# deepreinforce-ai/CUDA-L2

Measured on NVIDIA H100. Metric: HGEMM TFLOP/s, offline mode, per (M,N,K), higher is better.
Workload: dtype f16 x f16 -> f32 accumulate -> f16

## Files before the change

cuda_l2_b200/csrc/hgemm_sm90.cuh:

```cuda
#pragma once
#include <cuda.h>
#include <cuda_runtime.h>
#include <cstdint>

#include "hgemm_schedule.cuh"
#include "ptx_sm90.cuh"
#include "wgmma_sm90.cuh"


namespace b200 {

constexpr int kBlockKBytes = 128;
constexpr int kBlockK = 64;
constexpr int kWgmmaK = 16;
constexpr int kBlockM = 128;
constexpr int kNumThreads = 384;
constexpr int kEpiWarp0 = 4;
constexpr int kConsumerThreads = 256;
constexpr int kProducerRegs = 40;
constexpr int kConsumerRegs = 232;
constexpr int kSmemLimit = 232448;
enum KMode : int { kPlain = 0, kWorkspaceSplitK = 1, kClusterSplitK = 2, kStreamK = 3 };

template <int BN_, int STAGES_, int CTA_GROUP_, bool ACC_F32_, int CLUSTER_M_ = 1, int CLUSTER_N_ = 1, int M_REP_ = 1, bool BF16_ = false,
          bool E4M3_ = false>
struct Config {
  static constexpr int BN = BN_;
  static constexpr int CTA_GROUP = CTA_GROUP_;
  static constexpr bool ACC_F32 = ACC_F32_;
  static constexpr bool BF16 = BF16_;
  static_assert(!BF16_ || ACC_F32_, "bf16 operands accumulate in fp32");
  static constexpr bool E4M3 = E4M3_;
  static_assert(!E4M3_ || ACC_F32_, "e4m3 operands accumulate in fp32");
  static constexpr int OP_BYTES = E4M3_ ? 1 : 2;
  static constexpr int BLOCK_K = kBlockKBytes / OP_BYTES;
  static constexpr int CLUSTER_M = CLUSTER_M_;
  static constexpr int CLUSTER_N = CLUSTER_N_;
  static constexpr int MCAST_CTAS = CLUSTER_M * CLUSTER_N;
  static constexpr int MCAST_M = CTA_GROUP * CLUSTER_M;
  static constexpr int CLUSTER_CTAS = MCAST_M * CLUSTER_N;
  static constexpr int M_REP = M_REP_;
  static constexpr int CTA_M = kBlockM * M_REP;
  static constexpr int TILE_M = CTA_M * CTA_GROUP;
  static constexpr int A_BOX_ROWS = CTA_M / CLUSTER_N;
  static constexpr int B_BOX_ROWS = BN / MCAST_M;
  static constexpr int A_STAGE_BYTES = CTA_M * kBlockK * 2;
  static constexpr int B_STAGE_BYTES = BN * kBlockK * 2;
  static constexpr int STAGE_BYTES = A_STAGE_BYTES + B_STAGE_BYTES;
  static constexpr int EPI_N = BN < 64 ? BN : 64;
  static constexpr int EPI_CHUNKS = BN / EPI_N;
  static constexpr int EPI_ROWS = 16;
  static constexpr int NUM_THREADS = kNumThreads;
  static constexpr bool STREAM_K = CLUSTER_M_ * CLUSTER_N_ == 1 && BN_ >= 64 && M_REP_ == 1;
  static constexpr bool SPLIT_K = STREAM_K && CTA_GROUP_ == 1;
  static constexpr bool BLOCK_SCALED = false, BATCHED = false, GROUPED = false, ROW_MAJOR_B = false;
  using Cursor = NoBatches;
  static constexpr int EPI_BYTES = 8 * EPI_ROWS * 64 * 2;
  static constexpr int BAR_BYTES = 256;
  static constexpr int MAX_STAGES = (kSmemLimit - 1024 - EPI_BYTES - BAR_BYTES) / STAGE_BYTES;
  static constexpr int STAGES = STAGES_ < MAX_STAGES ? STAGES_ : MAX_STAGES;
  static constexpr int SMEM_BYTES = 1024  + STAGES * STAGE_BYTES + EPI_BYTES + BAR_BYTES;
  static_assert(BN == 32 || BN % 64 == 0, "tile N is 32 or a multiple of 64");
  static_assert(BN >= 32 && BN <= 256, "wgmma N constraints");
  static_assert(M_REP * BN <= 256, "register accumulators: at most 256 columns x 128 rows per consumer warpgroup");
  static_assert(CLUSTER_CTAS <= 8, "portable cluster size");
  static_assert(A_BOX_ROWS % 8 == 0 && B_BOX_ROWS % 8 == 0, "slices must cover whole 8-row swizzle atoms");
  static_assert(M_REP == 1 || M_REP == 2, "one or two 128-row blocks per CTA");
  static_assert(A_BOX_ROWS <= 256 && B_BOX_ROWS <= 256, "TMA box dimension limit");
  static_assert(STAGES >= 2, "the ring needs two stages");
  static_assert(SMEM_BYTES <= kSmemLimit, "exceeds 227 KB of shared memory");
  static_assert(A_STAGE_BYTES % 1024 == 0 && B_STAGE_BYTES % 1024 == 0, "swizzle-128B tiles need 1 KB alignment");
  static_assert(8 * (2 * STAGES + 1) <= BAR_BYTES, "barrier block too small");
};

constexpr int kMaxSplitTiles = 256;

template <class Base>
struct BlockScaled : Base {
  static constexpr bool BLOCK_SCALED = true;
  static_assert(Base::E4M3 && Base::M_REP * Base::BN <= 128, "block scales: e4m3, and room for two accumulator sets");
  static constexpr int SA_WINDOW_BYTES = Base::CTA_M * 4;
  static constexpr int SCALE_STAGE_BYTES = SA_WINDOW_BYTES + 16;
  static constexpr int MAX_STAGES =
      (kSmemLimit - 1024 - Base::EPI_BYTES - Base::BAR_BYTES) / (Base::STAGE_BYTES + SCALE_STAGE_BYTES);
  static constexpr int STAGES = Base::STAGES < MAX_STAGES ? Base::STAGES : MAX_STAGES;
  static constexpr int SMEM_BYTES = Base::SMEM_BYTES + STAGES * SCALE_STAGE_BYTES - (Base::STAGES - STAGES) * Base::STAGE_BYTES;
  static_assert(STAGES >= 2 && SMEM_BYTES <= kSmemLimit, "block-scaled ring does not fit");
};
template <class Cfg>
__host__ __device__ constexpr bool block_scaled() { return Cfg::BLOCK_SCALED; }

template <class Base>
struct Batched : Base {
  static constexpr bool BATCHED = true;
  using Cursor = BatchCursor;
  static_assert(!Base::E4M3, "batched: 16-bit operands, or block-scaled e4m3 (Batched<BlockScaled<...>>)");
};
template <class Base>
struct Batched<BlockScaled<Base>> : BlockScaled<Base> {
  static constexpr bool BATCHED = true;
  using Cursor = BatchCursor;
};
template <class Cfg>
__host__ __device__ constexpr bool batched() { return Cfg::BATCHED; }

template <class Base>
struct Grouped : Base {
  static constexpr bool GROUPED = true;
  using Cursor = GroupCursor;
  static_assert(!Base::E4M3, "grouped: 16-bit operands, or block-scaled e4m3 (Grouped<BlockScaled<...>>)");
};
template <class Base>
struct Grouped<BlockScaled<Base>> : BlockScaled<Base> {
  static constexpr bool GROUPED = true;
  using Cursor = GroupCursor;
  static constexpr int SA_WINDOW_BYTES = Base::CTA_M * 4 + 16;
  static constexpr int SCALE_STAGE_BYTES = SA_WINDOW_BYTES + 16;
  static constexpr int MAX_STAGES =
      (kSmemLimit - 1024 - Base::EPI_BYTES - Base::BAR_BYTES) / (Base::STAGE_BYTES + SCALE_STAGE_BYTES);
  static constexpr int STAGES = Base::STAGES < MAX_STAGES ? Base::STAGES : MAX_STAGES;
  static constexpr int SMEM_BYTES = Base::SMEM_BYTES + STAGES * SCALE_STAGE_BYTES - (Base::STAGES - STAGES) * Base::STAGE_BYTES;
  static_assert(STAGES >= 2 && SMEM_BYTES <= kSmemLimit, "grouped block-scaled ring does not fit");
  static_assert(Base::CTA_M % 4 == 0, "the scale window's shift is the group's");
};
template <class Cfg>
__host__ __device__ constexpr bool grouped() { return Cfg::GROUPED; }

template <class Base>
struct RowMajorB : Base {
  static constexpr bool ROW_MAJOR_B = true;
  static_assert(!Base::E4M3 && !Base::BLOCK_SCALED && !Base::BATCHED && !Base::GROUPED,
                "row-major B: the 2-D 16-bit kernels only");
  static_assert(Base::BN % 64 == 0, "row-major B: whole 64-column atom columns");
  static constexpr int B_ATOMS = Base::BN / 64;
  static constexpr int B_ATOM_BYTES = 64 * kBlockK * 2;
  static constexpr int B_K_ROWS = kBlockK / Base::MCAST_M;
  static_assert(B_K_ROWS % 8 == 0, "K slices of whole 8-row swizzle groups");
  static_assert(B_ATOMS * B_ATOM_BYTES == Base::B_STAGE_BYTES, "the stage holds the same bytes as the K-major one");
};
template <class Cfg>
__host__ __device__ constexpr bool row_major_b() { return Cfg::ROW_MAJOR_B; }

struct Scales { const float* a; const float* b; bool rowwise = false; };

template <class Cfg>
__device__ __forceinline__ float output_scale(const Scales& s) {
  if constexpr (Cfg::E4M3 && !block_scaled<Cfg>()) return s.rowwise ? 1.f : __fmul_rn(*s.a, *s.b);
  else return 1.f;
}

template <class Cfg>
__device__ __forceinline__ void scale_quad(float4& acc, float scale, const Scales& s, int gm, int gn) {
  if constexpr (Cfg::E4M3 && !block_scaled<Cfg>()) {
    if (s.rowwise) {
      const float sa = s.a[gm];
      const float4 sb = *reinterpret_cast<const float4*>(s.b + gn);
      acc.x = __fmul_rn(__fmul_rn(acc.x, sb.x), sa); acc.y = __fmul_rn(__fmul_rn(acc.y, sb.y), sa);
      acc.z = __fmul_rn(__fmul_rn(acc.z, sb.z), sa); acc.w = __fmul_rn(__fmul_rn(acc.w, sb.w), sa);
    } else {
      acc.x = __fmul_rn(acc.x, scale); acc.y = __fmul_rn(acc.y, scale);
      acc.z = __fmul_rn(acc.z, scale); acc.w = __fmul_rn(acc.w, scale);
    }
  }
}

struct RowwiseEpi { float sa_lo, sa_hi; const float* sb; };

__device__ __forceinline__ int frag_row(int lane, int p) { return (lane >> 2) + 8 * (p & 1); }
__device__ __forceinline__ int frag_col(int lane, int p) { return (p >> 1) * 8 + (lane & 3) * 2; }

template <class Cfg, class Reg, int NR>
__device__ __forceinline__ float2 acc_pair(const Reg (&d)[NR], int p) {
  if constexpr (Cfg::ACC_F32) {
    return make_float2(d[2 * p], d[2 * p + 1]);
  } else {
    const uint32_t v = d[p];
    const __half2 h = *reinterpret_cast<const __half2*>(&v);
    return make_float2(__low2float(h), __high2float(h));
  }
}
template <class Cfg, class Reg, int NR>
__device__ __forceinline__ uint32_t acc_packed(const Reg (&d)[NR], int p) {
  if constexpr (Cfg::ACC_F32) return ptx::pack_out_x2_rn<Cfg::BF16>(d[2 * p], d[2 * p + 1]);
  else return d[p];
}

template <class Cfg, class Reg, int NR>
__device__ __forceinline__ void epilogue_store_chunk(const Reg (&d)[NR], int chunk, uint32_t epi_buf, int lane,
                                                     const CUtensorMap* tmap_c, int col0, int row0, int M, int N,
                                                     const RowwiseEpi* rw = nullptr, int batch = 0,
                                                     __half* __restrict__ c_raw = nullptr) {
  using namespace ptx;
  constexpr int EN = Cfg::EPI_N;
  constexpr int PER_CHUNK = EN / 4;
  if (lane == 0) tma_store_wait_read<0>();
  __syncwarp();
  [[maybe_unused]] float2 sb_lane = make_float2(0.f, 0.f);
  [[maybe_unused]] float sbx = 0.f, sby = 0.f;
  if constexpr (Cfg::E4M3) {
    const int n = col0 + 2 * lane;
    if (rw && 2 * lane < EN && n < N) sb_lane = *reinterpret_cast<const float2*>(rw->sb + n);
  }
#pragma unroll
  for (int q = 0; q < PER_CHUNK; ++q) {
    uint32_t off = uint32_t(frag_row(lane, q) * (EN * 2) + frag_col(lane, q) * 2);
    off ^= (EN == 64 ? ((off >> 7) & 7u) : ((off >> 7) & 3u)) << 4;
    if constexpr (Cfg::E4M3) {
      if (rw) {
        if ((q & 1) == 0) {
          const int src = frag_col(lane, q) / 2;
          sbx = __shfl_sync(0xffffffffu, sb_lane.x, src);
          sby = __shfl_sync(0xffffffffu, sb_lane.y, src);
        }
        const float sa = (q & 1) ? rw->sa_hi : rw->sa_lo;
        const float2 v = acc_pair<Cfg>(d, chunk * PER_CHUNK + q);
        st_shared_b32(epi_buf + off, pack_out_x2_rn<Cfg::BF16>(__fmul_rn(__fmul_rn(v.x, sbx), sa),
                                                               __fmul_rn(__fmul_rn(v.y, sby), sa)));
        continue;
      }
    }
    st_shared_b32(epi_buf + off, acc_packed<Cfg>(d, chunk * PER_CHUNK + q));
  }
  fence_proxy_async_smem();
  __syncwarp();
  if constexpr (grouped<Cfg>()) {
    if (row0 + Cfg::EPI_ROWS > M) {
      constexpr int CPR = EN * 2 / 16;
#pragma unroll 1
      for (int i = lane; i < Cfg::EPI_ROWS * CPR; i += 32) {
        const int r = i / CPR, c = i % CPR;
        if (row0 + r < M && col0 + 8 * c < N) {
          uint32_t off = uint32_t(r * (EN * 2) + c * 16);
          off ^= (EN == 64 ? ((off >> 7) & 7u) : ((off >> 7) & 3u)) << 4;
          *reinterpret_cast<uint4*>(c_raw + size_t(row0 + r) * N + col0 + 8 * c) = ld_shared_v4_b32(epi_buf + off);
        }
      }
      return;
    }
  }
  if (lane == 0) {
    if (row0 < M && col0 < N) {
      if constexpr (batched<Cfg>()) tma_store_3d(tmap_c, epi_buf, col0, row0, batch);
      else tma_store_2d(tmap_c, epi_buf, col0, row0);
    }
    tma_store_commit();
  }
}

template <class Cfg, class Reg, int NR>
__device__ __forceinline__ void splitk_epilogue(const Reg (&d)[NR], int e, int row_base, int lane, int tile, int split,
                                                int splits, int m_base, int n0, int M, int N, float* __restrict__ ws,
                                                unsigned* __restrict__ ctr, __half* __restrict__ C,
                                                uint32_t red_smem, uint32_t red_bar, const Scales& scales) {
  using namespace ptx;
  constexpr int BN = Cfg::BN;
  float* slot = ws + (size_t(tile) * splits + split) * (kBlockM * BN);
#pragma unroll
  for (int p = 0; p < NR * (Cfg::ACC_F32 ? 1 : 2) / 2; ++p) {
    const float2 v = acc_pair<Cfg>(d, p);
    __stcg(reinterpret_cast<float2*>(slot + size_t(row_base + frag_row(lane, p)) * BN + frag_col(lane, p)), v);
  }
  __threadfence();
  asm volatile("bar.sync 1, %0;" ::"n"(kConsumerThreads) : "memory");
  if (e == 0) {
    asm volatile("red.release.gpu.global.add.u32 [%0], 1;" ::"l"(ctr + tile) : "memory");
    unsigned seen = 0, spins = 0;
    do {
      asm volatile("ld.acquire.gpu.global.u32 %0, [%1];" : "=r"(seen) : "l"(ctr + tile) : "memory");
      if (seen < unsigned(splits)) {
        __nanosleep(64);
        if (++spins > (1u << 24)) __trap();
      }
    } while (seen < unsigned(splits));
  }
  asm volatile("bar.sync 1, %0;" ::"n"(kConsumerThreads) : "memory");
  const int rows_per = (kBlockM + splits - 1) / splits;
  const int r0 = split * rows_per;
  const int r1 = min(kBlockM, r0 + rows_per);
  if (r0 < r1) {
    const uint32_t slice_bytes = uint32_t(r1 - r0) * BN * 4u;
    const float* tile_ws = ws + size_t(tile) * splits * (kBlockM * BN) + size_t(r0) * BN;
    if (e == 0) {
      fence_proxy_async_all();
      mbar_arrive_expect_tx(red_bar, slice_bytes * uint32_t(splits));
      for (int sp = 0; sp < splits; ++sp)
        bulk_load_1d(red_smem + uint32_t(sp) * slice_bytes, tile_ws + size_t(sp) * (kBlockM * BN), slice_bytes, red_bar);
    }
    mbar_wait(red_bar, 0);
    const float scale = output_scale<Cfg>(scales);
    constexpr int V = BN / 4;
    for (int i = e; i < (r1 - r0) * V; i += kConsumerThreads) {
      const int r = r0 + i / V, c4 = i % V;
      const int gm = m_base + r, gn = n0 + c4 * 4;
      if (gm >= M || gn >= N) continue;
      float4 acc = make_float4(0.f, 0.f, 0.f, 0.f);
      for (int sp = 0; sp < splits; ++sp) {
        const float4 p = ld_shared_v4f(red_smem + uint32_t(sp) * slice_bytes + uint32_t(i) * 16u);
        acc.x += p.x; acc.y += p.y; acc.z += p.z; acc.w += p.w;
      }
      scale_quad<Cfg>(acc, scale, scales, gm, gn);
      uint2 out;
      out.x = pack_out_x2_rn<Cfg::BF16>(acc.x, acc.y);
      out.y = pack_out_x2_rn<Cfg::BF16>(acc.z, acc.w);
      *reinterpret_cast<uint2*>(C + size_t(gm) * N + gn) = out;
    }
  }
  asm volatile("bar.sync 1, %0;" ::"n"(kConsumerThreads) : "memory");
  if (e == 0) {
    unsigned old;
    asm volatile("atom.acq_rel.gpu.global.add.u32 %0, [%1], 1;" : "=r"(old) : "l"(ctr + kMaxSplitTiles + tile) : "memory");
    if (old == unsigned(splits - 1)) {
      ctr[tile] = 0;
      ctr[kMaxSplitTiles + tile] = 0;
      __threadfence();
    }
  }
}

__host__ __device__ constexpr uint32_t cluster_partial_row_bytes(int bn) { return uint32_t(bn) * 4u + 16u; }

template <class Cfg, class Reg, int NR>
__device__ __forceinline__ void cluster_splitk_park(const Reg (&d)[NR], int row_base, int lane, uint32_t part_smem) {
  using namespace ptx;
#pragma unroll
  for (int p = 0; p < NR * (Cfg::ACC_F32 ? 1 : 2) / 2; ++p) {
    const float2 v = acc_pair<Cfg>(d, p);
    st_shared_v2f(part_smem + uint32_t(row_base + frag_row(lane, p)) * cluster_partial_row_bytes(Cfg::BN) +
                      uint32_t(frag_col(lane, p)) * 4u, v.x, v.y);
  }
}

template <class Cfg>
__device__ __forceinline__ void cluster_splitk_reduce(int e, int split, int splits, int m_base, int n0, int M, int N,
                                                      uint32_t part_smem, __half* __restrict__ C,
                                                      const Scales& scales) {
  using namespace ptx;
  constexpr int BN = Cfg::BN;
  constexpr int V = BN / 4;
  const float scale = output_scale<Cfg>(scales);
  const int rows_per = kBlockM / splits;
  const int r0 = split * rows_per;
  uint32_t peer[8];
#pragma unroll
  for (int p = 0; p < 8; ++p) peer[p] = (p < splits) ? mapa(part_smem, uint32_t(p)) : 0u;
  for (int i = e; i < rows_per * V; i += kConsumerThreads) {
    const int r = r0 + i / V, c4 = i % V;
    const int gm = m_base + r, gn = n0 + c4 * 4;
    if (gm >= M || gn >= N) continue;
    const uint32_t off = uint32_t(r) * cluster_partial_row_bytes(BN) + uint32_t(c4) * 16u;
    float4 acc = make_float4(0.f, 0.f, 0.f, 0.f);
#pragma unroll
    for (int p = 0; p < 8; ++p) {
      if (p < splits) {
        const float4 v = ld_dsmem_v4f(peer[p] + off);
        acc.x += v.x; acc.y += v.y; acc.z += v.z; acc.w += v.w;
      }
    }
    scale_quad<Cfg>(acc, scale, scales, gm, gn);
    uint2 out;
    out.x = pack_out_x2_rn<Cfg::BF16>(acc.x, acc.y);
    out.y = pack_out_x2_rn<Cfg::BF16>(acc.z, acc.w);
    *reinterpret_cast<uint2*>(C + size_t(gm) * N + gn) = out;
  }
}

constexpr int kMaxStreamKSlots = 160;
constexpr int kStreamKFlagsPerSlot = 8;

template <class Cfg>
struct StreamK {
  static constexpr int REGS = Cfg::ACC_F32 ? Cfg::BN / 2 : Cfg::BN / 4;
  static constexpr int R4 = REGS / 4;
  static constexpr int SLOT_U4 = R4 * kConsumerThreads;
  static_assert(REGS % 4 == 0, "register images move in uint4");
};

template <class Cfg, class Reg, int NR>
__device__ __forceinline__ void streamk_contribute(const Reg (&d)[NR], int t, int ew, int lane, uint4* __restrict__ ws,
                                                   unsigned* __restrict__ flags, int slot) {
  using namespace ptx;
  using SK = StreamK<Cfg>;
  uint4* base = ws + size_t(slot) * SK::SLOT_U4 + t;
#pragma unroll
  for (int i = 0; i < SK::R4; ++i) {
    uint32_t x[4];
#pragma unroll
    for (int c = 0; c < 4; ++c) {
      if constexpr (Cfg::ACC_F32) x[c] = __float_as_uint(d[4 * i + c]);
      else x[c] = d[4 * i + c];
    }
    st_global_cg_v4(base + i * kConsumerThreads, x[0], x[1], x[2], x[3]);
  }
  __threadfence();
  __syncwarp();
  if (lane == 0) st_release_gpu(flags + slot * kStreamKFlagsPerSlot + ew, 1u);
}

template <class Cfg, class Reg, int NR>
__device__ __forceinline__ void streamk_own(Reg (&d)[NR], int t, int ew, int lane, const uint4* __restrict__ ws,
                                            unsigned* __restrict__ flags, int slot0, int slot_stride, int n) {
  using namespace ptx;
  using SK = StreamK<Cfg>;
  if (lane == 0) {
    for (int p = 0; p < n; ++p) {
      const unsigned* f = flags + (slot0 + p * slot_stride) * kStreamKFlagsPerSlot + ew;
      unsigned spins = 0;
      while (ld_acquire_gpu(f) == 0u) {
        __nanosleep(64);
        if (++spins > (1u << 24)) __trap();
      }
    }
  }
  __syncwarp();
#pragma unroll
  for (int i = 0; i < SK::R4; ++i) {
    float f[Cfg::ACC_F32 ? 4 : 8];
#pragma unroll
    for (int c = 0; c < 4; ++c) {
      if constexpr (Cfg::ACC_F32) {
        f[c] = d[4 * i + c];
      } else {
        const uint32_t v = d[4 * i + c];
        const __half2 h = *reinterpret_cast<const __half2*>(&v);
        f[2 * c] = __low2float(h); f[2 * c + 1] = __high2float(h);
      }
    }
    for (int p = 0; p < n; ++p) {
      const uint4 v = ld_global_cg_v4(ws + size_t(slot0 + p * slot_stride) * SK::SLOT_U4 + size_t(i) * kConsumerThreads + t);
      const uint32_t x[4] = {v.x, v.y, v.z, v.w};
#pragma unroll
      for (int c = 0; c < 4; ++c) {
        if constexpr (Cfg::ACC_F32) {
          f[c] += __uint_as_float(x[c]);
        } else {
          const __half2 h = *reinterpret_cast<const __half2*>(&x[c]);
          f[2 * c] += __low2float(h); f[2 * c + 1] += __high2float(h);
        }
      }
    }
#pragma unroll
    for (int c = 0; c < 4; ++c) {
      if constexpr (Cfg::ACC_F32) d[4 * i + c] = f[c];
      else d[4 * i + c] = pack_out_x2_rn<false>(f[2 * c], f[2 * c + 1]);
    }
  }
  __syncwarp();
  if (lane == 0)
    for (int p = 0; p < n; ++p) flags[(slot0 + p * slot_stride) * kStreamKFlagsPerSlot + ew] = 0u;
}

template <class Cfg, int KMODE = kPlain>
__global__ void __launch_bounds__(kNumThreads, 1)
hgemm_tn_kernel(const __grid_constant__ CUtensorMap tmap_a,
                const __grid_constant__ CUtensorMap tmap_b,
                const __grid_constant__ CUtensorMap tmap_c,
                int M, int N, int K, int group_m,
                int splits_arg,
                int aux_arg,
                float* __restrict__ splitk_ws,
                unsigned* __restrict__ splitk_ctr,
                __half* __restrict__ c_raw,
                uint64_t hint_a, uint64_t hint_b,
                Scales scales                     ) {
  constexpr int BN = Cfg::BN;
  constexpr int STAGES = Cfg::STAGES;
  constexpr int EM = Cfg::MCAST_M;
  constexpr int CN = Cfg::CLUSTER_N;
  constexpr int MR = Cfg::M_REP;
  constexpr bool kSplit = (KMODE == kWorkspaceSplitK || KMODE == kClusterSplitK);
  static_assert(!kSplit || Cfg::SPLIT_K, "this configuration has no split-K epilogues");
  static_assert(KMODE != kStreamK || Cfg::STREAM_K, "this configuration has no stream-K epilogues");
  static_assert(!kSplit || (kBlockM + 32) * BN * 4 <= STAGES * Cfg::STAGE_BYTES, "split-K partials must fit the pipeline smem");
  const int splits = kSplit ? splits_arg : 1;
  const int sk_tiles = (KMODE == kStreamK) ? aux_arg : 0;
  using namespace ptx;

  extern __shared__ uint8_t smem_raw[];
  const uint32_t smem_base = (smem_u32(smem_raw) + 1023u) & ~1023u;
  const uint32_t smem_a = smem_base;
  const uint32_t smem_b = smem_a + STAGES * Cfg::A_STAGE_BYTES;
  const uint32_t smem_epi = smem_b + STAGES * Cfg::B_STAGE_BYTES;
  const uint32_t smem_bar = smem_epi + Cfg::EPI_BYTES;
  const uint32_t bar_full = smem_bar;
  const uint32_t bar_empty = bar_full + 8 * STAGES;
  const uint32_t bar_splitk = bar_empty + 8 * STAGES;
  constexpr bool kBlock = block_scaled<Cfg>();
  static_assert(!kBlock || KMODE == kPlain || KMODE == kClusterSplitK, "block scales: plain and cluster split-K only");
  [[maybe_unused]] const int ld_a = kBlock ? aux_arg : 0;
  [[maybe_unused]] const uint32_t smem_scales = smem_bar + Cfg::BAR_BYTES;
  constexpr bool kBatched = batched<Cfg>();
  constexpr bool kGrouped = grouped<Cfg>();
  constexpr bool kTileList = kBatched || kGrouped;
  constexpr bool kRowMajorB = row_major_b<Cfg>();
  static_assert(!kTileList || KMODE == kPlain, "batched / grouped: plain schedule only");
  [[maybe_unused]] const int num_batches = kTileList ? splits_arg : 1;
  [[maybe_unused]] const int* masked_m = kTileList ? reinterpret_cast<const int*>(splitk_ctr) : nullptr;
  using Cursor = typename Cfg::Cursor;

  const int warp = __shfl_sync(0xffffffffu, int(threadIdx.x) >> 5, 0);
  const int lane = threadIdx.x & 31;
  const uint32_t cluster_rank = (Cfg::CLUSTER_CTAS > 1) ? cluster_ctarank() : 0u;
  const int mi = int(cluster_rank) % EM;
  const int cn = int(cluster_rank) / EM;

  const int num_m_blocks = (M + Cfg::CTA_M * EM - 1) / (Cfg::CTA_M * EM);
  const int num_n_blocks = (N + BN * CN - 1) / (BN * CN);
  const int num_tiles = num_m_blocks * num_n_blocks;
  const int num_k_blocks = (K + Cfg::BLOCK_K - 1) / Cfg::BLOCK_K;
  const int num_workers = gridDim.x / Cfg::CLUSTER_CTAS;
  const int worker = blockIdx.x / Cfg::CLUSTER_CTAS;

  constexpr int kReleaseTargets = EM + CN - 1;
  if (threadIdx.x == 0) {
    for (int s = 0; s < STAGES; ++s) {
      mbar_init(bar_full + 8 * s, 1);
      mbar_init(bar_empty + 8 * s, 8 * kReleaseTargets);
    }
    mbar_init(bar_splitk, 1);
    fence_mbar_init();
    tma_prefetch_desc(&tmap_a);
    tma_prefetch_desc(&tmap_b);
    tma_prefetch_desc(&tmap_c);
  }
  if constexpr (Cfg::CLUSTER_CTAS > 1) cluster_sync_all(); else __syncthreads();

  grid_dependency_launch_dependents();
  grid_dependency_wait();

  if (warp < kEpiWarp0) {
    setmaxnreg_dec<kProducerRegs>();
    if (warp == 0) {
      uint16_t mask_a = 0, mask_b = 0;
#pragma unroll
      for (int j = 0; j < CN; ++j) mask_a |= uint16_t(1u << (mi + EM * j));
#pragma unroll
      for (int i = 0; i < EM; ++i) mask_b |= uint16_t(1u << (i + EM * cn));
      const uint32_t a_slice = uint32_t(cn) * (Cfg::A_BOX_ROWS * kBlockK * 2);
      const uint32_t b_slice = uint32_t(mi) * (Cfg::B_BOX_ROWS * kBlockK * 2);
      int stage = 0; uint32_t phase = 0;
      [[maybe_unused]] Cursor batches(masked_m, num_batches, M, Cfg::CTA_M * EM, num_n_blocks, group_m);
      WorkIter work(worker, num_workers, kTileList ? batches.total() : num_tiles, num_k_blocks, splits, sk_tiles);
      WorkUnit u;
      while (work.next(u)) {
        [[maybe_unused]] BatchTile bt{0, M, TileCoord{0, 0}};
        if constexpr (kTileList) bt = batches.locate(u.tile);
        const TileCoord tc = kTileList ? bt.tc : tile_coord(u.tile, num_m_blocks, num_n_blocks, group_m);
        const int m0 = (tc.m_blk * EM + mi) * Cfg::CTA_M + cn * Cfg::A_BOX_ROWS;
        const int n0 = (tc.n_blk * CN + cn) * BN + mi * Cfg::B_BOX_ROWS;
        [[maybe_unused]] int sa_m0 = (tc.m_blk * EM + mi) * Cfg::CTA_M;
        [[maybe_unused]] int sa_rows = kBlock ? max(0, min(Cfg::CTA_M, ld_a - sa_m0)) : 0;
        [[maybe_unused]] const int sb_n0 = (tc.n_blk * CN + cn) * BN;
        [[maybe_unused]] const float* sb_row = (kBlock && sb_n0 < N) ? scales.b + size_t(sb_n0 / 128) * num_k_blocks : nullptr;
        if constexpr (kBlock && kGrouped) {
          const int r0 = batches.start + sa_m0;
          sa_m0 = r0 & ~3;
          sa_rows = max(0, min(ld_a - sa_m0, ((r0 & 3) + Cfg::CTA_M + 3) & ~3));
        }
        if constexpr (kBlock && kTileList) {
          if (sb_row) sb_row += size_t(bt.batch) * ((N + 127) / 128) * num_k_blocks;
        }
        [[maybe_unused]] float sb_chunk = 0.f;
        for (int kb = u.kb0; kb < u.kb1; ++kb) {
          mbar_wait(bar_empty + 8 * stage, phase ^ 1);
          [[maybe_unused]] float sb_kb = 0.f;
          if constexpr (kBlock) {
            if (((kb - u.kb0) & 31) == 0) sb_chunk = (sb_row && kb + lane < u.kb1) ? sb_row[kb + lane] : 0.f;
            sb_kb = __shfl_sync(0xffffffffu, sb_chunk, (kb - u.kb0) & 31);
          }
          if (elect_one()) {
            const uint32_t full = bar_full + 8 * stage;
            if constexpr (kBlock) {
              const uint32_t sc = smem_scales + stage * Cfg::SCALE_STAGE_BYTES;
              st_shared_f32(sc + Cfg::SA_WINDOW_BYTES, sb_kb);
              mbar_arrive_expect_tx(full, Cfg::STAGE_BYTES + uint32_t(sa_rows) * 4u);
              if (sa_rows > 0) {
                if constexpr (kBatched)
                  bulk_load_1d(sc, scales.a + (size_t(bt.batch) * num_k_blocks + kb) * ld_a + sa_m0,
                               uint32_t(sa_rows) * 4u, full);
                else
                  bulk_load_1d(sc, scales.a + size_t(kb) * ld_a + sa_m0, uint32_t(sa_rows) * 4u, full);
              }
            } else {
              mbar_arrive_expect_tx(full, Cfg::STAGE_BYTES);
            }
            const uint32_t dst_a = smem_a + stage * Cfg::A_STAGE_BYTES + a_slice;
            const uint32_t dst_b = smem_b + stage * Cfg::B_STAGE_BYTES + b_slice;
            if constexpr (kBatched) {
              const int b = bt.batch;
              if constexpr (CN > 1) tma_load_3d_mcast_hint(dst_a, &tmap_a, full, kb * Cfg::BLOCK_K, m0, b, mask_a, hint_a);
              else tma_load_3d_hint(dst_a, &tmap_a, full, kb * Cfg::BLOCK_K, m0, b, hint_a);
              if constexpr (EM > 1) tma_load_3d_mcast_hint(dst_b, &tmap_b, full, kb * Cfg::BLOCK_K, n0, b, mask_b, hint_b);
              else tma_load_3d_hint(dst_b, &tmap_b, full, kb * Cfg::BLOCK_K, n0, b, hint_b);
            } else if constexpr (kGrouped) {
              const int ma = batches.start + m0, g = bt.batch;
              if constexpr (CN > 1) tma_load_2d_mcast_hint(dst_a, &tmap_a, full, kb * Cfg::BLOCK_K, ma, mask_a, hint_a);
              else tma_load_2d_hint(dst_a, &tmap_a, full, kb * Cfg::BLOCK_K, ma, hint_a);
              if constexpr (EM > 1) tma_load_3d_mcast_hint(dst_b, &tmap_b, full, kb * Cfg::BLOCK_K, n0, g, mask_b, hint_b);
              else tma_load_3d_hint(dst_b, &tmap_b, full, kb * Cfg::BLOCK_K, n0, g, hint_b);
            } else {
            if constexpr (CN > 1) tma_load_2d_mcast_hint(dst_a, &tmap_a, full, kb * Cfg::BLOCK_K, m0, mask_a, hint_a);
            else tma_load_2d_hint(dst_a, &tmap_a, full, kb * Cfg::BLOCK_K, m0, hint_a);
            if constexpr (kRowMajorB) {
              const uint32_t dst = smem_b + stage * Cfg::B_STAGE_BYTES + uint32_t(mi) * (Cfg::B_K_ROWS * kBlockKBytes);
              const int nb = (tc.n_blk * CN + cn) * BN, kr = kb * Cfg::BLOCK_K + mi * Cfg::B_K_ROWS;
#pragma unroll
              for (int j = 0; j < Cfg::B_ATOMS; ++j) {
                if constexpr (EM > 1)
                  tma_load_2d_mcast_hint(dst + j * Cfg::B_ATOM_BYTES, &tmap_b, full, nb + 64 * j, kr, mask_b, hint_b);
                else
                  tma_load_2d_hint(dst + j * Cfg::B_ATOM_BYTES, &tmap_b, full, nb + 64 * j, kr, hint_b);
              }
            } else {
            if constexpr (EM > 1) tma_load_2d_mcast_hint(dst_b, &tmap_b, full, kb * Cfg::BLOCK_K, n0, mask_b, hint_b);
            else tma_load_2d_hint(dst_b, &tmap_b, full, kb * Cfg::BLOCK_K, n0, hint_b);
            }
            }
          }
          __syncwarp();
          if (++stage == STAGES) { stage = 0; phase ^= 1; }
        }
      }
    }
    __syncwarp();
    if constexpr (KMODE == kClusterSplitK) {
      cluster_sync_all();
      cluster_sync_all();
    } else if constexpr (Cfg::CLUSTER_CTAS > 1) {
      cluster_sync_all();
    }
  } else {
    setmaxnreg_inc<kConsumerRegs>();
    using W = Wgmma<BN, Cfg::ACC_F32, Cfg::BF16 && !Cfg::E4M3, Cfg::E4M3, kRowMajorB>;
    constexpr int kDescBStep = kRowMajorB ? 16 * kBlockKBytes / 16 : 2;
    using Reg = typename W::Reg;
    constexpr int NR = W::kRegs;
    const int wg = warp / 4 - 1;
    const int wq = warp % 4;
    const int ew = warp - kEpiWarp0;
    const int t = int(threadIdx.x) - 128;
    const uint32_t epi_buf = smem_epi + uint32_t(ew) * (Cfg::EPI_ROWS * 64 * 2);
    [[maybe_unused]] int ck_m_base = 0, ck_n0 = 0, ck_split = 0;
    Reg acc[MR][NR];
#pragma unroll
    for (int r = 0; r < MR; ++r)
#pragma unroll
      for (int i = 0; i < NR; ++i) acc[r][i] = Reg(0);
    uint32_t empty_target = bar_empty;
    if constexpr (kReleaseTargets > 1) {
      uint32_t rank = cluster_rank;
      if (lane < EM) rank = uint32_t(lane + EM * cn);
      else if (lane < kReleaseTargets) { const int j = lane - EM; rank = uint32_t(mi + EM * (j < cn ? j : j + 1)); }
      empty_target = mapa(bar_empty, rank);
    }
    auto release = [&](int s) {
      __syncwarp();
      if constexpr (kReleaseTargets > 1) {
        if (lane < kReleaseTargets) mbar_arrive_cluster(empty_target + 8 * s);
      } else {
        if (lane == 0) mbar_arrive(bar_empty + 8 * s);
      }
    };
    int stage = 0; uint32_t phase = 0;
    [[maybe_unused]] Cursor batches(masked_m, num_batches, M, Cfg::CTA_M * EM, num_n_blocks, group_m);
    WorkIter work(worker, num_workers, kTileList ? batches.total() : num_tiles, num_k_blocks, splits, sk_tiles);
    WorkUnit u;
    while (work.next(u)) {
      if constexpr (kBlock) {
        static_assert(MR == 1 && Cfg::ACC_F32, "one 64-row block of fp32 accumulators per warpgroup");
        Reg part[NR];
        [[maybe_unused]] uint32_t sa_shift = 0;
        if constexpr (kGrouped) {
          batches.locate(u.tile);
          sa_shift = uint32_t(batches.start & 3) * 4u;
        }
        const uint32_t sa_off = uint32_t(wg * 64 + wq * 16 + (lane >> 2)) * 4u + sa_shift;
        for (int kb = u.kb0; kb < u.kb1; ++kb) {
          mbar_wait(bar_full + 8 * stage, phase);
          const uint64_t da = make_smem_desc(smem_a + stage * Cfg::A_STAGE_BYTES + uint32_t(wg) * (64 * kBlockK * 2));
          const uint64_t db = make_smem_desc(smem_b + stage * Cfg::B_STAGE_BYTES);
          reg_fence(part);
          wgmma_fence();
#pragma unroll
          for (int k = 0; k < kBlockK / kWgmmaK; ++k) W::mma(da + uint64_t(2 * k), db + uint64_t(2 * k), part, k > 0 ? 1u : 0u);
          wgmma_commit();
          wgmma_wait<0>();
          reg_fence(part);
          const uint32_t sc = smem_scales + stage * Cfg::SCALE_STAGE_BYTES;
          const float sb = ld_shared_f32(sc + Cfg::SA_WINDOW_BYTES);
          const float s_lo = __fmul_rn(ld_shared_f32(sc + sa_off), sb);
          const float s_hi = __fmul_rn(ld_shared_f32(sc + sa_off + 32u), sb);
          release(stage);
          if (kb == u.kb0) {
#pragma unroll
            for (int i = 0; i < NR; ++i) acc[0][i] = __fmul_rn(part[i], (i & 2) ? s_hi : s_lo);
          } else {
#pragma unroll
            for (int i = 0; i < NR; ++i) acc[0][i] = __fmaf_rn(part[i], (i & 2) ? s_hi : s_lo, acc[0][i]);
          }
          if (++stage == STAGES) { stage = 0; phase ^= 1; }
        }
        reg_fence(acc[0]);
      } else {
      int prev = -1;
      for (int kb = u.kb0; kb < u.kb1; ++kb) {
        mbar_wait(bar_full + 8 * stage, phase);
        const uint64_t da = make_smem_desc(smem_a + stage * Cfg::A_STAGE_BYTES + uint32_t(wg * MR) * (64 * kBlockK * 2));
        uint64_t db;
        if constexpr (kRowMajorB) db = make_smem_desc_mn(smem_b + stage * Cfg::B_STAGE_BYTES, 64 * kBlockKBytes);
        else db = make_smem_desc(smem_b + stage * Cfg::B_STAGE_BYTES);
#pragma unroll
        for (int r = 0; r < MR; ++r) reg_fence(acc[r]);
        wgmma_fence();
#pragma unroll
        for (int k = 0; k < kBlockK / kWgmmaK; ++k) {
#pragma unroll
          for (int r = 0; r < MR; ++r)
            W::mma(da + uint64_t(r * ((64 * kBlockK * 2) >> 4) + 2 * k), db + uint64_t(kDescBStep * k), acc[r],
                   (kb > u.kb0 || k > 0) ? 1u : 0u);
        }
        wgmma_commit();
        if constexpr (KMODE == kStreamK) wgmma_wait<0>();
        else wgmma_wait<1>();
#pragma unroll
        for (int r = 0; r < MR; ++r) reg_fence(acc[r]);
        if (prev >= 0) release(prev);
        prev = stage;
        if (++stage == STAGES) { stage = 0; phase ^= 1; }
      }
      wgmma_wait<0>();
#pragma unroll
      for (int r = 0; r < MR; ++r) reg_fence(acc[r]);
      release(prev);
      }

      const int tile = u.tile;
      [[maybe_unused]] BatchTile bt{0, M, TileCoord{0, 0}};
      if constexpr (kTileList) bt = batches.locate(tile);
      const TileCoord tc = kTileList ? bt.tc : tile_coord(tile, num_m_blocks, num_n_blocks, group_m);
      const int m_cta = (tc.m_blk * EM + mi) * Cfg::CTA_M;
      const int n0 = (tc.n_blk * CN + cn) * BN;
      [[maybe_unused]] uint4* ws4 = reinterpret_cast<uint4*>(splitk_ws);
      [[maybe_unused]] unsigned* sk_flags = splitk_ctr + 2 * kMaxSplitTiles;
      if constexpr (KMODE == kStreamK) {
        const int slot = worker * Cfg::CLUSTER_CTAS + int(cluster_rank);
        if (u.kb0 > 0) {
          streamk_contribute<Cfg>(acc[0], t, ew, lane, ws4, sk_flags, slot);
          continue;
        }
        if (u.kb1 < num_k_blocks) {
          const int n = streamk_contributors(worker, num_workers, sk_tiles * num_k_blocks, tile, num_k_blocks);
          streamk_own<Cfg>(acc[0], t, ew, lane, ws4, sk_flags, slot + Cfg::CLUSTER_CTAS, Cfg::CLUSTER_CTAS, n);
        }
      }
      if constexpr (KMODE == kClusterSplitK) {
        asm volatile("bar.sync 1, %0;" ::"n"(kConsumerThreads) : "memory");
        cluster_splitk_park<Cfg>(acc[0], wg * 64 + wq * 16, lane, smem_a);
        ck_m_base = m_cta; ck_n0 = n0; ck_split = worker - tile * splits;
      } else if constexpr (KMODE == kWorkspaceSplitK) {
        splitk_epilogue<Cfg>(acc[0], t, wg * 64 + wq * 16, lane, tile, worker - tile * splits, splits, m_cta, n0, M, N,
                             splitk_ws, splitk_ctr, c_raw, smem_a, bar_splitk, scales);
      } else {
        if constexpr (Cfg::E4M3 && !kBlock) {
          if (scales.rowwise) {
#pragma unroll
            for (int r = 0; r < MR; ++r) {
              const int row0 = m_cta + (wg * MR + r) * 64 + wq * 16;
              const int ra = row0 + (lane >> 2), rb = ra + 8;
              const RowwiseEpi rw{ra < M ? scales.a[ra] : 0.f, rb < M ? scales.a[rb] : 0.f, scales.b};
#pragma unroll
              for (int j = 0; j < Cfg::EPI_CHUNKS; ++j)
                epilogue_store_chunk<Cfg>(acc[r], j, epi_buf, lane, &tmap_c, n0 + j * Cfg::EPI_N, row0, M, N, &rw);
            }
            continue;
          }
          const float scale = output_scale<Cfg>(scales);
#pragma unroll
          for (int r = 0; r < MR; ++r)
#pragma unroll
            for (int i = 0; i < NR; ++i) acc[r][i] = __fmul_rn(acc[r][i], scale);
#pragma unroll
          for (int r = 0; r < MR; ++r) reg_fence(acc[r]);
        }
#pragma unroll
        for (int r = 0; r < MR; ++r) {
          const int row0 = m_cta + (wg * MR + r) * 64 + wq * 16;
#pragma unroll
          for (int j = 0; j < Cfg::EPI_CHUNKS; ++j) {
            if constexpr (kGrouped)
              epilogue_store_chunk<Cfg>(acc[r], j, epi_buf, lane, &tmap_c, n0 + j * Cfg::EPI_N, batches.start + row0,
                                        batches.end, N, nullptr, 0, c_raw);
            else
              epilogue_store_chunk<Cfg>(acc[r], j, epi_buf, lane, &tmap_c, n0 + j * Cfg::EPI_N, row0,
                                        kBatched ? bt.rows : M, N, nullptr, bt.batch);
          }
        }
      }
    }
    if (lane == 0) tma_store_wait_read<0>();
    __syncwarp();
    if constexpr (KMODE == kClusterSplitK) {
      cluster_sync_all();
      cluster_splitk_reduce<Cfg>(t, ck_split, splits, ck_m_base, ck_n0, M, N, smem_a, c_raw, scales);
      __syncwarp();
      cluster_sync_all();
    } else if constexpr (Cfg::CLUSTER_CTAS > 1) {
      cluster_sync_all();
    }
  }
}

}
```

Before: 730.7.

## Defer last epilogue chunk store into next tile's first mainloop iteration

For plain fp16 GEMM configs, the last output chunk of each tile is packed into registers rather than stored right away. It is written to shared memory and issued as a TMA store after the first WGMMA batch of the next work unit is committed, or after the loop ends. This is meant to hide the final epilogue store and its wait behind the next tile's tensor-core work. In exchange it holds extra live registers across the mainloop, which adds register pressure, and it puts a TMA store wait inside the K loop.

```diff
diff --git a/cuda_l2_b200/csrc/hgemm_sm90.cuh b/cuda_l2_b200/csrc/hgemm_sm90.cuh
--- a/cuda_l2_b200/csrc/hgemm_sm90.cuh
+++ b/cuda_l2_b200/csrc/hgemm_sm90.cuh
@@ -247,6 +247,40 @@
   }
 }
 
+template <class Cfg, int KMODE>
+__host__ __device__ constexpr bool carries_output() {
+  return KMODE == kPlain && !Cfg::E4M3 && !block_scaled<Cfg>() && !batched<Cfg>() && !grouped<Cfg>() && !row_major_b<Cfg>();
+}
+template <class Cfg>
+struct Carry {
+  static constexpr int LAST = Cfg::M_REP * Cfg::EPI_CHUNKS - 1;
+  static constexpr int REGS = Cfg::EPI_N / 4;
+};
+
+template <class Cfg>
+__device__ __forceinline__ void store_carried_chunk(const uint32_t (&packed)[Carry<Cfg>::REGS], uint32_t epi_buf,
+                                                    int lane, const CUtensorMap* tmap_c, int n0, int row0, int M, int N) {
+  using namespace ptx;
+  constexpr int EN = Cfg::EPI_N;
+  constexpr int PER_CHUNK = Carry<Cfg>::REGS;
+  const int col0 = n0 + (Carry<Cfg>::LAST % Cfg::EPI_CHUNKS) * EN;
+  row0 += (Carry<Cfg>::LAST / Cfg::EPI_CHUNKS) * 64;
+  if (lane == 0) tma_store_wait_read<0>();
+  __syncwarp();
+#pragma unroll
+  for (int q = 0; q < PER_CHUNK; ++q) {
+    uint32_t off = uint32_t(frag_row(lane, q) * (EN * 2) + frag_col(lane, q) * 2);
+    off ^= (EN == 64 ? ((off >> 7) & 7u) : ((off >> 7) & 3u)) << 4;
+    st_shared_b32(epi_buf + off, packed[q]);
+  }
+  fence_proxy_async_smem();
+  __syncwarp();
+  if (lane == 0) {
+    if (row0 < M && col0 < N) tma_store_2d(tmap_c, epi_buf, col0, row0);
+    tma_store_commit();
+  }
+}
+
 template <class Cfg, class Reg, int NR>
 __device__ __forceinline__ void splitk_epilogue(const Reg (&d)[NR], int e, int row_base, int lane, int tile, int split,
                                                 int splits, int m_base, int n0, int M, int N, float* __restrict__ ws,
@@ -661,6 +695,9 @@
       }
     };
     int stage = 0; uint32_t phase = 0;
+    constexpr bool kCarry = carries_output<Cfg, KMODE>();
+    [[maybe_unused]] uint32_t packed[kCarry ? Carry<Cfg>::REGS : 1];
+    [[maybe_unused]] int carry_n0 = -1, carry_row0 = 0;
     [[maybe_unused]] Cursor batches(masked_m, num_batches, M, Cfg::CTA_M * EM, num_n_blocks, group_m);
     WorkIter work(worker, num_workers, kTileList ? batches.total() : num_tiles, num_k_blocks, splits, sk_tiles);
     WorkUnit u;
@@ -719,6 +756,12 @@
                    (kb > u.kb0 || k > 0) ? 1u : 0u);
         }
         wgmma_commit();
+        if constexpr (kCarry) {
+          if (carry_n0 >= 0) {
+            store_carried_chunk<Cfg>(packed, epi_buf, lane, &tmap_c, carry_n0, carry_row0, M, N);
+            carry_n0 = -1;
+          }
+        }
         if constexpr (KMODE == kStreamK) wgmma_wait<0>();
         else wgmma_wait<1>();
 #pragma unroll
@@ -781,20 +824,36 @@
 #pragma unroll
           for (int r = 0; r < MR; ++r) reg_fence(acc[r]);
         }
-#pragma unroll
-        for (int r = 0; r < MR; ++r) {
-          const int row0 = m_cta + (wg * MR + r) * 64 + wq * 16;
-#pragma unroll
-          for (int j = 0; j < Cfg::EPI_CHUNKS; ++j) {
-            if constexpr (kGrouped)
-              epilogue_store_chunk<Cfg>(acc[r], j, epi_buf, lane, &tmap_c, n0 + j * Cfg::EPI_N, batches.start + row0,
-                                        batches.end, N, nullptr, 0, c_raw);
-            else
-              epilogue_store_chunk<Cfg>(acc[r], j, epi_buf, lane, &tmap_c, n0 + j * Cfg::EPI_N, row0,
-                                        kBatched ? bt.rows : M, N, nullptr, bt.batch);
+        if constexpr (kCarry) {
+          constexpr int LAST = Carry<Cfg>::LAST;
+          carry_n0 = n0;
+          carry_row0 = m_cta + wg * MR * 64 + wq * 16;
+#pragma unroll
+          for (int c = 0; c < LAST; ++c)
+            epilogue_store_chunk<Cfg>(acc[c / Cfg::EPI_CHUNKS], c % Cfg::EPI_CHUNKS, epi_buf, lane, &tmap_c,
+                                      n0 + (c % Cfg::EPI_CHUNKS) * Cfg::EPI_N, carry_row0 + (c / Cfg::EPI_CHUNKS) * 64, M, N);
+#pragma unroll
+          for (int q = 0; q < Carry<Cfg>::REGS; ++q)
+            packed[q] = acc_packed<Cfg>(acc[LAST / Cfg::EPI_CHUNKS], (LAST % Cfg::EPI_CHUNKS) * Carry<Cfg>::REGS + q);
+        } else {
+#pragma unroll
+          for (int r = 0; r < MR; ++r) {
+            const int row0 = m_cta + (wg * MR + r) * 64 + wq * 16;
+#pragma unroll
+            for (int j = 0; j < Cfg::EPI_CHUNKS; ++j) {
+              if constexpr (kGrouped)
+                epilogue_store_chunk<Cfg>(acc[r], j, epi_buf, lane, &tmap_c, n0 + j * Cfg::EPI_N, batches.start + row0,
+                                          batches.end, N, nullptr, 0, c_raw);
+              else
+                epilogue_store_chunk<Cfg>(acc[r], j, epi_buf, lane, &tmap_c, n0 + j * Cfg::EPI_N, row0,
+                                          kBatched ? bt.rows : M, N, nullptr, bt.batch);
+            }
           }
         }
       }
+    }
+    if constexpr (kCarry) {
+      if (carry_n0 >= 0) store_carried_chunk<Cfg>(packed, epi_buf, lane, &tmap_c, carry_n0, carry_row0, M, N);
     }
     if (lane == 0) tma_store_wait_read<0>();
     __syncwarp();
```

Result: no change. 737.6, median of 6 (+1.0%).
